# siyuanwu99/pred-occ-planner

Hardware: AMD Instinct MI355X
Metric: replans/sec (SOGM update + QP: full replan = SOGM update + A* + corridors + QP + deconfliction), 128-agent batch per GPU, 200x200x200x20 voxel grid; aggregate over all agents (higher is better)
Workload: dtype f32 occupancy / f64 planning; 1 GPU; 128 agents/GPU x 1 GPU, 200x200x200x20 SOGM, sim_fkpcp-style moving cylinders, batched ADMM QP (BASELINE configs[2] per GPU); agents_total=128, cloud_points=622040, cylinders=555, map_input_staleness_ticks=0, parallelism=agents sharded x1, 1 all-gather/tick, exchange=local, sogm_grids_per_agent=3, sogm_reset=sparse (logged 32-byte sectors), sogm_cell_order=2x2x2 tiles, map_update=at the start of the tick

## Files before the change

### pred-occ-planner_amd/csrc/sogm_qp.hip

```cpp
#include <hip/hip_runtime.h>

#include <cstdlib>

#include "../../include/sogm_detmath.h"
#include "sogm_planner.hpp"
#include "sogm_qp_layout.hpp"

#include <type_traits>

namespace sogm {
namespace {

#define QP_NMAX (15 * SOGM_MAX_PIECES)
#define QP_NT 512
#define QP_K1_DOUBLES (15 * QP_FAST_MAX_PIECES * (QP_BW + 1))

__device__ const double OSQP_INFTY  = 1e30;
__device__ const double MIN_SCALING = 1e-04, MAX_SCALING = 1e+04;
__device__ const double RHO_MIN = 1e-06, RHO_TOL = 1e-04, RHO_EQ_OVER_RHO_INEQ = 1e03;

__device__ inline double dabs(double x) { return x < 0 ? -x : x; }
__device__ inline double dmax(double a, double b) { return a > b ? a : b; }
__device__ inline double limit_scaling(double v) {
  v = v < MIN_SCALING ? 1.0 : v;
// ... 47 lines not shown
  v += dpp_ctrl_t<0x4E>(v);
  v += dpp_ctrl_t<0x141>(v);
  v += dpp_ctrl_t<0x140>(v);
  return (read_lane(v, 0) + read_lane(v, 16)) + (read_lane(v, 32) + read_lane(v, 48));
}
__device__ inline double block_max(double v, double *s_red) {
  v = wave_max(v);
  __syncthreads();
  if ((threadIdx.x & 63) == 0) s_red[threadIdx.x >> 6] = v;
  __syncthreads();
  return dmax(dmax(dmax(s_red[0], s_red[1]), dmax(s_red[2], s_red[3])),
              dmax(dmax(s_red[4], s_red[5]), dmax(s_red[6], s_red[7])));
}

static_assert(row_bytes('S', true) == (3 + 1) * sizeof(double) && row_bytes('G', true) == sizeof(double), "carve_rows: hot arrays");
static_assert(row_bytes('G', false) == (QP_ELL + 8) * sizeof(double) + 2 * QP_ELL * sizeof(int) &&
                  row_bytes('S', false) == 5 * sizeof(double) + sizeof(int),
              "carve_rows: cold arrays");
__device__ inline void carve_rows(Rows &R, char *hot, char *cold, int G, int S) {
  double *h = (double *)hot;
  R.sval = h;  h += (size_t)S * 3;
  R.sw = h;    h += S;
  R.gw = h;
  double *d = (double *)cold;
  R.gval = d;  d += (size_t)G * QP_ELL;
  R.gl = d;    d += G;
  R.gu = d;    d += G;
  R.grho = d;  d += G;
  R.gE = d;    d += G;
  R.gz = d;    d += G;
  R.gy = d;    d += G;
  R.gdy = d;   d += G;
  R.grinv = d; d += G;
  R.su = d;    d += S;
  R.sE = d;    d += S;
  R.sz = d;    d += S;
  R.sy = d;    d += S;
  R.sdy = d;   d += S;
  int *q = (int *)d;
  R.gcol = q;  q += (size_t)G * QP_ELL;
  R.sc0 = q;   q += S;
  R.cidx = q;
}

#define dpp_quad(v, ctrl) dpp_ctrl_t<ctrl>(v)

__device__ inline int launder(int v) {
  asm volatile("" : "+v"(v));
  return v;
}

__device__ inline double &KB(double *Kb, int i, int j) { return Kb[i * (QP_BW + 1) + (i - j)]; }

}

__device__ __forceinline__ void qp_solve_agent(const SogmPlannerParams &pp, const SogmQpSettings &qs,
                                               const QpWorkspace &ws, const QpConst &qc, const QpIO &io,
                                               int ablate_arg, int agent) {
#ifdef SOGM_QP_ABLATE_BUILD
  const int ablate = ablate_arg;
#else
  constexpr int ablate = 0;
  (void)ablate_arg;
#endif
  const int tid = threadIdx.x, lane = tid & 63, wave = tid >> 6;
  const long long dbg_t0 = wall_clock64(), dbg_clk0 = clock64();
  long long       dbg_refac = 0, dbg_check = 0, dbg_f1 = 0, dbg_f2 = 0, dbg_f3 = 0, dbg_k1 = 0, dbg_k2 = 0;
  int             dbg_nrefac = 0, dbg_ncheck = 0;
  const int M = io.npoly[agent];
  if (M <= 0 || M > SOGM_MAX_PIECES) {
    if (tid == 0) {
      io.out_status[agent] = -100;
      io.out_iters[agent]  = 0;
    }
    return;
  }
  const int MF = pp.max_faces;
  const int n  = 15 * M;

  extern __shared__ __attribute__((aligned(16))) char qp_smem[];
  const bool use_blocks = M <= QP_FAST_MAX_PIECES;
  __shared__ double s_ginv[QP_NMAX];
  __shared__ __attribute__((aligned(16))) double s_xt[QP_NMAX];
  __shared__ double s_x[QP_NMAX], s_D[QP_NMAX], s_Dt[QP_NMAX];
  __shared__ __attribute__((aligned(16))) double s_cn[QP_NMAX];
  __shared__ double s_red[8];
  __shared__ double s_T[2][225];
  __shared__ double s_red12[96];
  __shared__ double s_sc[16];
  __shared__ int    s_off[SOGM_MAX_PIECES + 1];
  __shared__ int    s_nf[SOGM_MAX_PIECES];
  __shared__ int    s_cnt[QP_NMAX + 1];
  __shared__ int    s_cptr[QP_NMAX + 1];
  __shared__ int    s_flag;

  if (tid == 0) {
    int acc = 0;
    for (int i = 0; i < M; ++i) {
      const int f = io.nfaces[agent * SOGM_MAX_PIECES + i];
      s_off[i]    = acc;
      s_nf[i]     = f;
      acc += 5 * f;
    }
    s_off[M] = acc;
  }
  __syncthreads();
// ... 234 lines not shown
      }
      R.gE[r] *= et;
    }
    for (int s = tid; s < S; s += QP_NT) {
      double      *v  = R.sval + (size_t)s * 3;
      const double mx = __builtin_fmax(__builtin_fmax(__builtin_fabs(v[0]), __builtin_fabs(v[1])), __builtin_fabs(v[2]));
      const double et = 1.0 / sogm_det::sqrt_rn(limit_scaling(mx));
      const int    c0 = R.sc0[s];
      v[0] *= et * s_Dt[c0];
      v[1] *= et * s_Dt[c0 + 1];
      v[2] *= et * s_Dt[c0 + 2];
      R.sE[s] *= et;
    }
    for (int jq = launder(tid); jq < 4 * n; jq += QP_NT) {
      const int     j = jq >> 2, q = jq & 3, b15 = (j / 15) * 15;
      double       *Pb = s_P + (j / 15) * 225 + j % 15;
      const double  dj = s_Dt[j];
      double        mx = 0;
      for (int i = q; i < 15; i += 4) {
        const double v = (Pb[i * 15] * ct_prev) * (s_Dt[b15 + i] * dj);
        Pb[i * 15]     = v;
        mx             = __builtin_fmax(mx, __builtin_fabs(v));
      }
      mx = __builtin_fmax(mx, dpp_quad(mx, 0xB1));
      mx = __builtin_fmax(mx, dpp_quad(mx, 0x4E));
      if (q == 0) {
        s_cn[j] = mx;
        s_D[j] *= dj;
      }
    }
    __syncthreads();
    if (tid == 0) {
      double mean = 0;
      for (int j = 0; j < n; ++j) mean += s_cn[j];
      double c_temp = mean / n;
      c_temp        = dmax(c_temp, limit_scaling(0.0));
      c_temp        = limit_scaling(c_temp);
      s_sc[0]       = 1.0 / c_temp;
    }
    __syncthreads();
    ct_prev = s_sc[0];
    c_scale *= ct_prev;
  }
  for (int i = tid; i < M * 225; i += QP_NT) s_P[i] *= ct_prev;
  for (int r = tid; r < G; r += QP_NT) {
    R.gl[r] *= R.gE[r];
    R.gu[r] *= R.gE[r];
  }
  for (int s = tid; s < S; s += QP_NT) R.su[s] *= R.sE[s];
  const double cinv = 1.0 / c_scale;
  __syncthreads();
  const long long dbg_s2 = wall_clock64() - dbg_t0;

  double rho_cur = qs.rho;
  double rinv_cur = 1.0 / rho_cur;
  double    kinv[30] = {};
  auto   set_rho = [&]() {
    const int tid = launder((int)threadIdx.x), lane = tid & 63, wave = tid >> 6;
    (void)lane;
    (void)wave;
    for (int r = tid; r < G; r += QP_NT) {
      const double lo = R.gl[r], hi = R.gu[r];
      double       v;
      if (lo < -OSQP_INFTY * MIN_SCALING && hi > OSQP_INFTY * MIN_SCALING)
        v = RHO_MIN;
      else if (hi - lo < RHO_TOL)
        v = RHO_EQ_OVER_RHO_INEQ * rho_cur;
      else
        v = rho_cur;
      R.grho[r]  = v;
      R.grinv[r] = 1.0 / v;
    }
    for (int s = tid; s < S; s += QP_NT) R.sw[s] = rho_cur * R.sz[s] - R.sy[s];
    __syncthreads();
  };
  auto build_K1 = [&]() {
    const int tid = launder((int)threadIdx.x);
    for (int e = tid; e < n * (QP_BW + 1); e += QP_NT) {
      const int i = e / (QP_BW + 1), dlt = e % (QP_BW + 1), j = i - dlt;
      double    s = 0.0;
      if (j >= 0) {
        for (int a = s_cptr[i]; a < s_cptr[i + 1]; ++a) {
          const int    en = R.cidx[a], r = en >> 3;
          const double vi = R.gval[(size_t)r * QP_ELL + (en & 7)];
          const double mr = R.gu[r] - R.gl[r] < RHO_TOL ? RHO_EQ_OVER_RHO_INEQ : 1.0;
          for (int k = 0; k < QP_ELL; ++k)
            if (R.gcol[(size_t)r * QP_ELL + k] == j) s += vi * mr * R.gval[(size_t)r * QP_ELL + k];
        }
        if (i / 3 == j / 3) {
          COL_DECODE(i)
          const int jd = j % 3;
          for (int f = 0; f < nface; ++f) {
            const double *v = R.sval + (size_t)(sbase + 5 * f) * 3;
            s += v[pd] * v[jd];
          }
        }
      }
      k1w[e] = s;
    }
    __threadfence_block();
    __syncthreads();
  };
  auto factor = [&]() __attribute__((always_inline)) -> bool {
    const int tid = launder((int)threadIdx.x), lane = tid & 63, wave = tid >> 6;
    (void)lane;
    (void)wave;
    if constexpr (FAST) {
      const long long dbg_fa = wall_clock64();
      for (int e = tid; e < 2 * M * 225; e += QP_NT) {
        const int which = e >= M * 225 ? 1 : 0, ee = e - which * M * 225;
        const int b = ee / 225, r = (ee % 225) / 15, c = ee % 15;
        int       i = b * 15 + r, j = (b - which) * 15 + c;
        double    s = 0.0;
        if (j >= 0) {
          if (i < j) {
            const int t_ = i;
            i            = j;
            j            = t_;
          }
          if (i / 15 == j / 15) s = s_P[(i / 15) * 225 + (i % 15) * 15 + (j % 15)];
          if (i == j) s += qs.sigma;
          if (i - j <= QP_BW) s = __builtin_fma(rho_cur, k1r[i * (QP_BW + 1) + (i - j)], s);
        }
        (which ? s_V : s_Dv)[ee] = s;
      }
      if (tid == 0) s_flag = 1;
      __syncthreads();
      const long long dbg_fb = wall_clock64();
      dbg_f1 += dbg_fb - dbg_fa;
      const int  er = (tid % 225) / 15, ec = tid % 15;
      const bool el = tid < 225;
      const int  hi_ = er > ec ? er : ec, lo_ = er > ec ? ec : er;
      for (int i = 0; i < M; ++i) {
        double a = 0.0;
        if (i > 0) {
          if (el) {
            const double *Or = s_V + i * 225 + er * 15, *Dc = s_Dv + (i - 1) * 225 + ec;
            double        t  = 0.0;
#pragma unroll
            for (int k = 0; k < 15; ++k) t = __builtin_fma(Or[k], Dc[k * 15], t);
            s_T[0][tid] = t;
          }
          __syncthreads();
          if (el) {
            const double *Tr = s_T[0] + hi_ * 15, *Oc = s_V + i * 225 + lo_ * 15;
            double        t  = s_Dv[i * 225 + hi_ * 15 + lo_];
#pragma unroll
            for (int k = 0; k < 15; ++k) t = __builtin_fma(-Tr[k], Oc[k], t);
            a = t;
          }
          __syncthreads();
          if (el) s_V[i * 225 + tid] = s_T[0][tid];
        } else if (el) {
// ... 279 lines not shown
    }
    if (!(ablate & 64))
    for (int j = tid; j < n; j += QP_NT) {
      double        s  = 0;
      const double *Pb = s_P + (j / 15) * 225 + (j % 15) * 15;
      const int     b0 = (j / 15) * 15;
      for (int k = 0; k < 15; ++k) s += Pb[k] * s_x[b0 + k];
      const double a  = col_sum_y(j);
      const double dj = 1.0 / s_D[j];
      m[3]            = dmax(m[3], dabs(dj * (s + a)));
      m[4]            = dmax(m[4], dabs(dj * s));
      m[5]            = dmax(m[5], dabs(dj * a));
      m[9]            = dmax(m[9], dabs(s + a));
      m[10]           = dmax(m[10], dabs(s));
      m[11]           = dmax(m[11], dabs(a));
    }
    if (!(ablate & 128))
#pragma unroll
    for (int k = 0; k < 12; ++k) m[k] = wave_max(m[k]);
    __syncthreads();
    if (lane == 0) {
      double *o = s_red12 + wave * 12;
#pragma unroll
      for (int k = 0; k < 12; ++k) o[k] = m[k];
    }
    __syncthreads();
    if (tid < 12) {
      double v = s_red12[tid];
      for (int w = 1; w < QP_NT / 64; ++w) v = dmax(v, s_red12[12 * w + tid]);
      s_sc[tid < 6 ? tid : tid + 2] = tid == 3 ? v * cinv : v;
    }
    if (tid == 12) s_sc[6] = s_sc[14] = 0.0;
    __syncthreads();
  };

  double *const h_sv = (double *)(qp_smem + head);
  double *const h_sw = h_sv + (size_t)S * 3;
  double *const h_gw = h_sw + S;
  double rs[24];
  int    ri[QP_ELL];
#define gv(k) rs[k]
#define gc(k) ri[k]
#define g_rho rs[6]
#define g_rinv rs[7]
#define g_lo rs[8]
#define g_hi rs[9]
#define g_z rs[10]
#define g_y rs[11]
#define sv(u, d) rs[6 * (u) + (d)]
#define s_hi(u) rs[6 * (u) + 3]
#define s_zr(u) rs[6 * (u) + 4]
#define s_yr(u) rs[6 * (u) + 5]
#define s_c(u) ri[u]
  double cv[2], xj = 0.0;
  int    cr[2];
#pragma unroll
  for (int k = 0; k < 24; ++k) rs[k] = 0.0;
#pragma unroll
  for (int k = 0; k < QP_ELL; ++k) ri[k] = 0;
  cv[0] = cv[1] = 0.0;
  cr[0] = cr[1] = 0;
  const bool grole = tid < 256;
  const bool grow = tid < G, ccol = tid < 4 * n;
  int        fj_sv = 0, fj_sw = 0, fj_n = 0;
  auto fast_load = [&]() __attribute__((always_inline)) {
    const int t  = launder(tid);
    const int tg = grow ? t : 0;
    if (grole) {
#pragma unroll
      for (int k = 0; k < QP_ELL; ++k) {
        const int    c = R.gcol[(size_t)tg * QP_ELL + k];
        const double v = R.gval[(size_t)tg * QP_ELL + k];
        gc(k)          = (c < 0 || !grow) ? 0 : c;
        gv(k)          = (c < 0 || !grow) ? 0.0 : v;
      }
      g_lo = R.gl[tg];
      g_hi = R.gu[tg];
      g_z  = R.gz[tg];
      g_y  = R.gy[tg];
#pragma unroll
      for (int k = 12; k < 24; ++k) rs[k] = 0.0;
    } else {
#pragma unroll
      for (int u = 0; u < 4; ++u) {
        const int  sr = (t - 256) + 256 * u;
        const bool ok = sr < S;
        const int  sc = ok ? sr : 0;
        const double a0 = R.sval[(size_t)sc * 3 + 0], a1 = R.sval[(size_t)sc * 3 + 1], a2 = R.sval[(size_t)sc * 3 + 2];
        const double hi = R.su[sc], z = R.sz[sc], y = R.sy[sc];
        const int    c0 = R.sc0[sc];
        sv(u, 0) = ok ? a0 : 0.0;
        sv(u, 1) = ok ? a1 : 0.0;
        sv(u, 2) = ok ? a2 : 0.0;
        s_hi(u)  = ok ? hi : 0.0;
        s_zr(u)  = ok ? z : 0.0;
        s_yr(u)  = ok ? y : 0.0;
        s_c(u)   = ok ? c0 : 0;
      }
      ri[4] = ri[5] = 0;
    }
    {
      const int j = ccol ? t >> 2 : 0, q = t & 3;
#pragma unroll
      for (int e = 0; e < 2; ++e) {
        const int    qq = s_cptr[j] + q + 4 * e;
        const bool   ok = ccol && qq < s_cptr[j + 1];
        const int    en = R.cidx[ok ? qq : s_cptr[j]];
        const double v  = R.gval[(size_t)(en >> 3) * QP_ELL + (en & 7)];
        cr[e]           = ok ? en >> 3 : 0;
        cv[e]           = ok ? v : 0.0;
      }
      COL_DECODE(j)
      fj_sv = (sbase + 5 * q) * 3 + pd;
      fj_sw = sbase + 5 * q;
      fj_n  = ccol ? (nface - q + 3) >> 2 : 0;
      xj    = s_x[j];
    }
  };
  auto fast_rho = [&]() __attribute__((always_inline)) {
    const int t  = launder(tid);
    const int tg = grow ? t : 0;
    if (grole) {
      g_rho  = R.grho[tg];
      g_rinv = R.grinv[tg];
      if (grow) h_gw[t] = g_rho * g_z - g_y;
    }
  };
  double *const c_sy = (double *)qp_smem + (size_t)M * 225;
  double *const c_gy = c_sy + S;
  double *const c_red = c_gy + G;
  auto fast_stage_y = [&]() __attribute__((always_inline)) {
    const int t = launder(tid);
    if (grole) {
      if (grow) c_gy[t] = g_y;
    } else {
#pragma unroll
      for (int u = 0; u < 4; ++u) {
        const int sr = (t - 256) + 256 * u;
        if (sr < S) c_sy[sr] = s_yr(u);
      }
    }
    if (ccol && (t & 3) == 0) s_x[t >> 2] = xj;
    __syncthreads();
  };
  auto fast_spill = [&]() __attribute__((always_inline)) {
    const int t = launder(tid);
    if (grole) {
      if (grow) {
        R.gz[t] = g_z;
        R.gy[t] = g_y;
      }
    } else {
#pragma unroll
      for (int u = 0; u < 4; ++u) {
        const int sr = (t - 256) + 256 * u;
        if (sr < S) {
          R.sz[sr] = s_zr(u);
          R.sy[sr] = s_yr(u);
        }
      }
    }
    if (ccol && (t & 3) == 0) s_x[t >> 2] = xj;
    __syncthreads();
  };

  auto cert_stage1 = [&]() {
    const int tid = launder((int)threadIdx.x), lane = tid & 63, wave = tid >> 6;
    double    ndy = 0, lhs = 0;
    for (int r = tid; r < G; r += QP_NT) {
      const double d = R.gdy[r];
      ndy            = dmax(ndy, dabs(R.gE[r] * d));
      lhs += R.gu[r] * (d > 0 ? d : 0) + R.gl[r] * (d < 0 ? d : 0);
    }
    for (int s = tid; s < S; s += QP_NT) {
      const double d = R.sdy[s] > 0.0 ? R.sdy[s] : 0.0;
      R.sdy[s]       = d;
      ndy            = dmax(ndy, dabs(R.sE[s] * d));
      lhs += R.su[s] * d;
    }
    ndy = block_max(ndy, s_red);
    lhs = wave_sum(lhs);
    __syncthreads();
    if (lane == 0) s_red[wave] = lhs;
    __syncthreads();
    if (tid == 0) {
      s_sc[7]  = ndy;
      s_sc[15] = ((s_red[0] + s_red[1]) + (s_red[2] + s_red[3])) + ((s_red[4] + s_red[5]) + (s_red[6] + s_red[7]));
    }
    __syncthreads();
  };
  auto primal_infeasible = [&](double eps_inf) -> bool {
    const int tid = launder((int)threadIdx.x);
    if constexpr (!FAST) cert_stage1();
    const double ndy = s_sc[7], lhs = s_sc[15];
    if (!(ndy > eps_inf)) return false;
    if (!(lhs < -eps_inf * ndy)) return false;
    double na = 0;
    if constexpr (FAST) {
      if (ccol) {
        const int     j = tid >> 2;
        double        a = __builtin_fma(cv[1], R.gdy[cr[1]], cv[0] * R.gdy[cr[0]]);
        const double *fvp = h_sv + fj_sv, *fyp = R.sdy + fj_sw;
        const double *fv0 = fvp, *fy0 = fyp;
#pragma unroll 1
        for (int i0 = 0; i0 < fj_n; i0 += 4, fvp += 240, fyp += 80) {
          double av[4], bv[4];
#pragma unroll
          for (int u = 0; u < 4; ++u) {
            const bool ok = i0 + u < fj_n;
            av[u]         = *(ok ? fvp + 60 * u : fv0);
            bv[u]         = *(ok ? fyp + 20 * u : fy0);
            bv[u]         = ok ? bv[u] : 0.0;
          }
#pragma unroll
          for (int u = 0; u < 4; ++u) a = __builtin_fma(av[u], bv[u], a);
        }
        a += dpp_quad(a, 0xB1);
        a += dpp_quad(a, 0x4E);
        na = dabs((1.0 / s_D[j]) * a);
      }
    } else {
      for (int j = tid; j < n; j += QP_NT) {
        double a = 0;
        for (int q = s_cptr[j]; q < s_cptr[j + 1]; ++q) {
          const int en = R.cidx[q], r = en >> 3;
          a += R.gval[(size_t)r * QP_ELL + (en & 7)] * R.gdy[r];
        }
        COL_DECODE(j)
        for (int f = 0; f < nface; ++f) {
          const int sr = sbase + 5 * f;
          a += R.sval[(size_t)sr * 3 + pd] * R.sdy[sr];
        }
        na = dmax(na, dabs((1.0 / s_D[j]) * a));
      }
    }
    na = block_max(na, s_red);
    __syncthreads();
    return na < eps_inf * ndy;
  };

  auto fast_residuals = [&]() __attribute__((always_inline)) {
    const int  t = launder(tid), lane = t & 63, wave = t >> 6;
    const bool f32 = qs.residual_fp32 != 0;
    auto fab = [](double x) __attribute__((always_inline)) { return __builtin_fabs(x); };
    auto fmx = [](double a, double b) __attribute__((always_inline)) { return __builtin_fmax(a, b); };
    double    v[10];
#pragma unroll
    for (int k = 0; k < 10; ++k) v[k] = 0.0;
    if (grole) {
      double xg[QP_ELL];
#pragma unroll
      for (int k = 0; k < QP_ELL; ++k) xg[k] = s_x[gc(k)];
      const int    tg = grow ? t : 0;
      const double e = R.gE[tg], d = R.gdy[tg];
      double       ax = 0.0;
#pragma unroll
      for (int k = 0; k < QP_ELL; ++k) ax += gv(k) * xg[k];
      if (grow) {
        const double r_ = fab(ax - g_z), n_ = fmx(fab(ax), fab(g_z));
        const double ei = 1.0 / e;
        v[0] = f32 ? (double)((float)r_ / (float)e) : ei * r_;
        v[1] = f32 ? (double)((float)n_ / (float)e) : ei * n_;
        v[2] = r_;
        v[3] = n_;
        v[8] = fab(e * d);
        v[9] = g_hi * (d > 0 ? d : 0) + g_lo * (d < 0 ? d : 0);
      }
    } else {
      double se[4], sd[4];
#pragma unroll
      for (int u = 0; u < 4; ++u) {
        const int sr = (t - 256) + 256 * u, sc = sr < S ? sr : 0;
        se[u] = R.sE[sc];
        sd[u] = R.sdy[sc];
      }
#pragma unroll
      for (int u = 0; u < 4; ++u) {
        if (256 * u >= S) continue;
        const int    sr = (t - 256) + 256 * u;
        const bool   ok = sr < S;
        const double x0 = s_x[s_c(u)], x1 = s_x[s_c(u) + 1], x2 = s_x[s_c(u) + 2];
        const double e = se[u], dr_ = sd[u];
        double       ax = 0.0;
        ax += sv(u, 0) * x0;
        ax += sv(u, 1) * x1;
        ax += sv(u, 2) * x2;
        if (ok) {
          const double d  = dr_ > 0.0 ? dr_ : 0.0;
          R.sdy[sr]       = d;
          const double r_ = fab(ax - s_zr(u)), n_ = fmx(fab(ax), fab(s_zr(u)));
          const double ei = 1.0 / e;
          v[0] = fmx(v[0], f32 ? (double)((float)r_ / (float)e) : ei * r_);
          v[1] = fmx(v[1], f32 ? (double)((float)n_ / (float)e) : ei * n_);
          v[2] = fmx(v[2], r_);
          v[3] = fmx(v[3], n_);
          v[8] = fmx(v[8], fab(e * d));
          v[9] += s_hi(u) * d;
        }
      }
    }
    if (ccol) {
      const int     j = t >> 2, q = t & 3, b0 = (j / 15) * 15;
      const double *Pb = s_P + (j / 15) * 225 + (j % 15) * 15;
      double        pk[4], xk[4], yg[2];
#pragma unroll
      for (int u = 0; u < 4; ++u) {
        const int k = q + 4 * u, kk = k < 15 ? k : 0;
        pk[u]       = Pb[kk];
        xk[u]       = s_x[b0 + kk];
      }
#pragma unroll
      for (int e = 0; e < 2; ++e) yg[e] = c_gy[cr[e]];
      double        s_ = 0.0, a_ = 0.0;
      {
        const double *fvp = h_sv + fj_sv, *fyp = c_sy + fj_sw;
        const double *fv0 = fvp, *zero = s_xt + 127;
#pragma unroll 1
        for (int i0 = 0; i0 < fj_n; i0 += 4, fvp += 240, fyp += 80) {
          double a[4], b[4];
#pragma unroll
          for (int u = 0; u < 4; ++u) {
            const bool ok = i0 + u < fj_n;
            a[u]          = *(ok ? fvp + 60 * u : fv0);
            b[u]          = *(ok ? fyp + 20 * u : zero);
          }
          __builtin_amdgcn_sched_barrier(0);
#pragma unroll
          for (int u = 0; u < 4; ++u) a_ = __builtin_fma(a[u], b[u], a_);
        }
      }
#pragma unroll
      for (int u = 0; u < 4; ++u) s_ = __builtin_fma(q + 4 * u < 15 ? pk[u] : 0.0, xk[u], s_);
#pragma unroll
      for (int e = 0; e < 2; ++e) a_ = __builtin_fma(cv[e], yg[e], a_);
      s_ += dpp_quad(s_, 0xB1);
      a_ += dpp_quad(a_, 0xB1);
      s_ += dpp_quad(s_, 0x4E);
      a_ += dpp_quad(a_, 0x4E);
      if (q == 0) {
        const double dj = s_D[j], di = 1.0 / dj;
        const double r_ = fab(s_ + a_), n_ = fmx(fab(s_), fab(a_));
        v[4] = f32 ? (double)((float)r_ / (float)dj) : di * r_;
        v[5] = f32 ? (double)((float)n_ / (float)dj) : di * n_;
        v[6] = r_;
        v[7] = n_;
      }
    }
    if (f32) {
#pragma unroll
      for (int k = 0; k < 9; ++k) {
        float fv = (float)v[k];
        if ((double)fv < v[k]) fv = __int_as_float(__float_as_int(fv) + 1);
        v[k] = (double)fv;
      }
    }
#pragma unroll
    for (int k = 0; k < 9; ++k) {
      double x = v[k];
      x        = __builtin_fmax(x, dpp_ctrl_t<0xB1>(x));
      x        = __builtin_fmax(x, dpp_ctrl_t<0x4E>(x));
      x        = __builtin_fmax(x, dpp_ctrl_t<0x141>(x));
      v[k]     = __builtin_fmax(x, dpp_ctrl_t<0x140>(x));
    }
    {
      double x = v[9];
      x += dpp_ctrl_t<0xB1>(x);
      x += dpp_ctrl_t<0x4E>(x);
      x += dpp_ctrl_t<0x141>(x);
      v[9] = x + dpp_ctrl_t<0x140>(x);
    }
    if ((lane & 15) == 0) {
      double *o = c_red + (wave * 4 + (lane >> 4)) * 10;
#pragma unroll
      for (int k = 0; k < 10; ++k) o[k] = v[k];
    }
    __syncthreads();
    if (t < 40) {
      const int     k = t >> 2, pq = t & 3;
      const double *o = c_red + (size_t)(8 * pq) * 10 + k;
      double        r_;
      if (k == 9) {
        r_ = ((o[0] + o[10]) + (o[20] + o[30])) + ((o[40] + o[50]) + (o[60] + o[70]));
        r_ += dpp_quad(r_, 0xB1);
        r_ += dpp_quad(r_, 0x4E);
      } else {
        r_ = __builtin_fmax(__builtin_fmax(__builtin_fmax(o[0], o[10]), __builtin_fmax(o[20], o[30])),
                            __builtin_fmax(__builtin_fmax(o[40], o[50]), __builtin_fmax(o[60], o[70])));
        r_ = __builtin_fmax(r_, dpp_quad(r_, 0xB1));
        r_ = __builtin_fmax(r_, dpp_quad(r_, 0x4E));
      }
      const int slot = k == 0 ? 0 : k == 1 ? 1 : k == 2 ? 8 : k == 3 ? 9 : k == 4 ? 3 : k == 5 ? 4 : k == 6 ? 11 : k == 7 ? 12 : k == 8 ? 7 : 15;
      if (pq == 0) s_sc[slot] = k == 4 ? r_ * cinv : r_;
    }
    if (t >= 64 && t < 70)
      s_sc[t == 64 ? 2 : t == 65 ? 5 : t == 66 ? 6 : t == 67 ? 10 : t == 68 ? 13 : 14] = 0.0;
    __syncthreads();
  };

  set_rho();
  if constexpr (FAST) build_K1();
  const long long dbg_s3 = wall_clock64() - dbg_t0;
  bool chol_ok = factor();
  const long long dbg_setup = wall_clock64() - dbg_t0;
  int  status = -2, iter = 0;
  if (!chol_ok) status = -7;
  if constexpr (FAST) {
    fast_load();
    fast_rho();
    __syncthreads();
  }

  int cj_q0 = 0, cj_q1 = 0, cj_sbase = 0, cj_nface = 0, cj_pd = 0;
  if (tid < n) {
    COL_DECODE(tid)
    cj_q0    = s_cptr[tid];
    cj_q1    = s_cptr[tid + 1];
    cj_sbase = sbase;
    cj_nface = nface;
    cj_pd    = pd;
  }
  double alpha = qs.alpha, oma = 1.0 - qs.alpha, sigma_v = qs.sigma;
  asm volatile("" : "+v"(alpha), "+v"(oma), "+v"(sigma_v));
  const double *xtv   = FAST ? s_cn : s_xt;
  for (int j = n + tid; j < 128; j += QP_NT) s_xt[j] = 0.0;
  __syncthreads();
  auto iteration = [&](auto store_tag, auto ns_tag) __attribute__((always_inline)) {
      constexpr bool STORE = decltype(store_tag)::value;
      constexpr int  NS    = decltype(ns_tag)::value;
      (void)NS;
      if constexpr (FAST) {
        if (!(ablate & 1) && ccol) {
          double w[2];
#pragma unroll
          for (int e = 0; e < 2; ++e) w[e] = h_gw[cr[e]];
          double        p   = 0.0;
          const double *fvp = h_sv + fj_sv, *fwp = h_sw + fj_sw;
          const double *fv0 = fvp, *zero = s_xt + 127;
#pragma unroll 1
          for (int i0 = 0; i0 < fj_n; i0 += 4, fvp += 240, fwp += 80) {
            double a[4], b[4];
#pragma unroll
            for (int u = 0; u < 4; ++u) {
              const bool ok = i0 + u < fj_n;
              a[u]          = *(ok ? fvp + 60 * u : fv0);
              b[u]          = *(ok ? fwp + 20 * u : zero);
            }
            __builtin_amdgcn_sched_barrier(0);
#pragma unroll
            for (int u = 0; u < 4; ++u) p = __builtin_fma(a[u], b[u], p);
          }
#pragma unroll
          for (int e = 0; e < 2; ++e) p = __builtin_fma(cv[e], w[e], p);
          p += dpp_quad(p, 0xB1);
          p += dpp_quad(p, 0x4E);
          if ((tid & 3) == 0) s_xt[launder(tid) >> 2] = __builtin_fma(sigma_v, xj, p);
        }
      } else
      if (!(ablate & 1))
      if (tid < n) {
        const int j = tid;
        double    s = qs.sigma * s_x[j];
        for (int q = cj_q0; q < cj_q1; ++q) {
          const int en = R.cidx[q], r = en >> 3;
          s += R.gval[(size_t)r * QP_ELL + (en & 7)] * (R.grho[r] * R.gz[r] - R.gy[r]);
        }
        const double *sv = R.sval + (size_t)cj_sbase * 3 + cj_pd;
        const double *sw = R.sw + cj_sbase;
        for (int f = 0; f < cj_nface; ++f) s += sv[(size_t)15 * f] * sw[5 * f];
        s_xt[j] = s;
      }
      __syncthreads();
      if (!(ablate & 2)) solveK();
      if constexpr (FAST) {
        if (!(ablate & 12)) {
          const int    t   = launder(tid);
          const double xtj = xtv[ccol ? t >> 2 : 0];
          if (grole) {
            double xg[QP_ELL];
#pragma unroll
            for (int k = 0; k < QP_ELL; ++k) xg[k] = xtv[gc(k)];
            __builtin_amdgcn_sched_barrier(0);
            double s = gv(0) * xg[0];
#pragma unroll
            for (int k = 1; k < QP_ELL; ++k) s = __builtin_fma(gv(k), xg[k], s);
            const double zr = __builtin_fma(alpha, s, oma * g_z);
            double       v  = __builtin_fma(g_rinv, g_y, zr);
            v               = __builtin_fmin(__builtin_fmax(v, g_lo), g_hi);
            g_z             = v;
            const double d  = g_rho * (zr - v);
            g_y             = g_y + d;
            if (grow) {
              h_gw[t] = __builtin_fma(g_rho, v, -g_y);
              if constexpr (STORE) R.gdy[t] = d;
            }
          } else {
            double xs[NS][3];
#pragma unroll
            for (int u = 0; u < NS; ++u) {
              xs[u][0] = xtv[s_c(u)];
              xs[u][1] = xtv[s_c(u) + 1];
              xs[u][2] = xtv[s_c(u) + 2];
            }
            __builtin_amdgcn_sched_barrier(0);
#pragma unroll
            for (int u = 0; u < NS; ++u) {
              double ax = sv(u, 0) * xs[u][0];
              ax              = __builtin_fma(sv(u, 1), xs[u][1], ax);
              ax              = __builtin_fma(sv(u, 2), xs[u][2], ax);
              const double zr = __builtin_fma(alpha, ax, oma * s_zr(u));
              double       v  = __builtin_fma(rinv_cur, s_yr(u), zr);
              v               = __builtin_fmin(v, s_hi(u));
              s_zr(u)         = v;
              const double d  = rho_cur * (zr - v);
              const double yn = s_yr(u) + d;
              s_yr(u)         = yn;
              const int sr    = (t - 256) + 256 * u;
              if (u + 1 < NS || sr < S) {
                h_sw[sr] = __builtin_fma(rho_cur, v, -yn);
                if constexpr (STORE) R.sdy[sr] = d;
              }
            }
          }
          xj = __builtin_fma(alpha, xtj, oma * xj);
        }
        __syncthreads();
      } else {
      if (!(ablate & 4))
      for (int r = tid; r < G; r += QP_NT) {
        double s = 0;
        for (int k = 0; k < QP_ELL; ++k) {
          const int c = R.gcol[(size_t)r * QP_ELL + k];
          if (c >= 0) s += R.gval[(size_t)r * QP_ELL + k] * xtv[c];
        }
        const double rho = R.grho[r], yr = R.gy[r];
        const double zr  = alpha * s + (1.0 - alpha) * R.gz[r];
        double       v   = zr + R.grinv[r] * yr;
        const double lo = R.gl[r], hi = R.gu[r];
        v               = v < lo ? lo : (v > hi ? hi : v);
        R.gz[r]         = v;
        const double d  = rho * (zr - v);
        R.gdy[r]        = d;
        R.gy[r]         = yr + d;
      }
      if (!(ablate & 8))
      for (int s = tid; s < S; s += QP_NT) {
        const int     c0 = R.sc0[s];
        const double *vv = R.sval + (size_t)s * 3;
        double        ax = 0;
        ax += vv[0] * xtv[c0];
        ax += vv[1] * xtv[c0 + 1];
        ax += vv[2] * xtv[c0 + 2];
        const double yr = R.sy[s];
        const double zr = alpha * ax + (1.0 - alpha) * R.sz[s];
        double       v  = zr + rinv_cur * yr;
        const double hi = R.su[s];
        v               = v > hi ? hi : v;
        R.sz[s]         = v;
        const double d  = rho_cur * (zr - v);
        R.sdy[s]        = d;
        const double yn = yr + d;
        R.sy[s]         = yn;
        R.sw[s]         = rho_cur * v - yn;
      }
      for (int j = tid; j < n; j += QP_NT) s_x[j] = alpha * xtv[j] + (1.0 - alpha) * s_x[j];
      __syncthreads();
      }
  };
  int adapt_left = qs.adaptive_rho_interval, check_left = qs.check_termination;
  bool finished = !chol_ok;
  if (chol_ok) {
    const int max_iter = qs.max_iter, adapt_iv = qs.adaptive_rho_interval, check_iv = qs.check_termination;
// ... 89 lines not shown
      } else {
        residuals();
      }
      const double eps_prim = qs.eps_abs * 10 + qs.eps_rel * 10 * dmax(s_sc[1], s_sc[2]);
      const double eps_dual =
          qs.eps_abs * 10 + qs.eps_rel * 10 * cinv * dmax(dmax(s_sc[4], s_sc[5]), s_sc[6]);
      const bool p_ok = s_sc[0] < eps_prim;
      if (p_ok && s_sc[3] < eps_dual)
        status = 2;
      else if (!p_ok && primal_infeasible(1e-4 * 10))
        status = 3;
      else
        status = -2;
    }
  }
  __syncthreads();
  double *out = io.out_cpts + (size_t)agent * SOGM_MAX_PIECES * 15;
  for (int j = tid; j < SOGM_MAX_PIECES * 15; j += QP_NT) out[j] = j < n ? s_D[j] * s_x[j] : 0.0;
  if (tid == 0) {
    io.out_status[agent] = status;
    io.out_iters[agent]  = iter;
    if (ws.dbg) {
      long long *o = ws.dbg + (size_t)agent * SOGM_QP_STAT_N;
      o[SOGM_QP_STAT_FACTOR_ASM]    = dbg_f1;
      o[SOGM_QP_STAT_FACTOR_FWD]    = dbg_f2;
      o[SOGM_QP_STAT_FACTOR_BWD]    = dbg_f3;
      o[SOGM_QP_STAT_SHADER_CLOCKS] = clock64() - dbg_clk0;
      o[SOGM_QP_STAT_CHECK_STAGE]   = dbg_k1;
      o[SOGM_QP_STAT_CHECK_RESID]   = dbg_k2;
      o[SOGM_QP_STAT_TOTAL]         = wall_clock64() - dbg_t0;
      o[SOGM_QP_STAT_SETUP_SPLIT]   = dbg_s1 | (dbg_s2 << 20) | (dbg_s3 << 40);
      o[SOGM_QP_STAT_SETUP]         = dbg_setup;
      o[SOGM_QP_STAT_REFAC]         = dbg_refac;
      o[SOGM_QP_STAT_N_REFAC]       = dbg_nrefac;
      o[SOGM_QP_STAT_CHECK]         = dbg_check;
      o[SOGM_QP_STAT_N_CHECK]       = dbg_ncheck;
      o[SOGM_QP_STAT_ITERS]         = iter;
      o[SOGM_QP_STAT_PATH]          = (FAST ? 1 : 0) | (rows_in_lds ? 2 : 0);
    }
  }
#undef gv
#undef gc
#undef g_rho
#undef g_rinv
#undef g_lo
#undef g_hi
#undef g_z
#undef g_y
#undef sv
#undef s_hi
#undef s_zr
#undef s_yr
#undef s_c
  };
  using std::false_type;
  using std::true_type;
  if (rows_in_lds) {
    Rows R;
    carve_rows(R, qp_smem + head, qp_smem + head + rows_hot_bytes(G, S), G, S);
    if (fast)
      body(R, true_type{});
    else
      body(R, false_type{});
  } else {
    char *scr = ws.scratch + (size_t)agent * ws.scratch_stride;
    Rows  R;
    carve_rows(R, fast ? qp_smem + head : scr, scr + rows_hot_bytes(G, S), G, S);
    if (fast)
      body(R, true_type{});
    else
      body(R, false_type{});
  }
}

__global__ __launch_bounds__(QP_NT) void k_qp(SogmPlannerParams pp, SogmQpSettings qs, QpWorkspace ws,
                                            QpConst qc, const double *__restrict__ start_pva,
                                            const double *__restrict__ goal_pv,
                                            const double *__restrict__ polys,
                                            const int32_t *__restrict__ nfaces,
                                            const int32_t *__restrict__ npoly,
                                            double *__restrict__ out_cpts,
                                            int32_t *__restrict__ out_status,
                                            int32_t *__restrict__ out_iters, int ablate_arg, int agent0) {
  const QpIO io{.start_pva = start_pva, .goal_pv = goal_pv, .polys = polys, .nfaces = nfaces, .npoly = npoly,
                .out_cpts = out_cpts, .out_status = out_status, .out_iters = out_iters};
  qp_solve_agent(pp, qs, ws, qc, io, ablate_arg, blockIdx.x + agent0);
}

__global__ __launch_bounds__(QP_NT) void k_qp_flow(SogmPlannerParams pp, SogmQpSettings qs, QpWorkspace ws,
                                                 QpConst qc, FlowCtl fc, QpIO io, int ablate_arg, int n_agents) {
  __shared__ int s_agent;
  if (threadIdx.x == 0) atomicAdd(&fc.hdr[FLOW_Q_RESIDENT], 1);
  for (;;) {
    if (threadIdx.x == 0) {
      int       a = -1;
      const int k = atomicAdd(&fc.hdr[FLOW_Q_TICKET], 1);
      if (k < n_agents) a = wait_at_least<WaitQpItem, false>(&fc.hdr[FLOW_ERR], fc.q_ready + k, 0);
      s_agent = a;
    }
    __syncthreads();
    const int agent = __builtin_amdgcn_readfirstlane(s_agent);
    if (agent < 0) break;
    __threadfence();
    if (threadIdx.x == 0) fc.ts[agent * 8 + 4] = wall_clock64();
    qp_solve_agent(pp, qs, ws, qc, io, ablate_arg, agent);
    __syncthreads();
// ... 69 lines not shown
```

### pred-occ-planner_amd/csrc/sogm_qp_layout.hpp

```cpp
#pragma once
#include <cstddef>
#include "../../include/sogm_abi.h"
#ifdef __HIPCC__
#include <hip/hip_runtime.h>
#define QP_HD __host__ __device__ __forceinline__
#define QP_HDI __host__ __device__ inline
#else
#define QP_HD inline
#define QP_HDI inline
#endif

namespace sogm {

constexpr int QP_BW  = 17;
constexpr int QP_ELL = 6;

struct QpShape {
  int M, n;
  int R1, R3, R4;
  int G, S;
  QP_HD QpShape(int pieces, int faces)
      : M(pieces), n(15 * pieces), R1(3 * (pieces + 1)), R3(9 * (pieces + 1)), R4(R3 + 12 * pieces), G(R4 + 9 * pieces),
        S(5 * faces) {}
};

#define QP_ROW_ARRAYS(X)                                                                                      \
  X(sval, S, 3, double, true)                                                            \
  X(sw, S, 1, double, true)          \
  X(gw, G, 1, double, true)                                                 \
  X(gval, G, QP_ELL, double, false)                                                           \
  X(gl, G, 1, double, false)                                                                                  \
  X(gu, G, 1, double, false)                                                                                  \
  X(grho, G, 1, double, false)                                                                                \
  X(gE, G, 1, double, false)                                                                                  \
  X(gz, G, 1, double, false)                                                                                  \
  X(gy, G, 1, double, false)                                                                                  \
  X(gdy, G, 1, double, false)                                                                                 \
  X(grinv, G, 1, double, false)                                               \
  X(su, S, 1, double, false)                                                                                  \
  X(sE, S, 1, double, false)                                                                                  \
  X(sz, S, 1, double, false)                                                                                  \
  X(sy, S, 1, double, false)                                                                                  \
  X(sdy, S, 1, double, false)                                                                                 \
  X(gcol, G, QP_ELL, int, false)                                              \
  X(sc0, S, 1, int, false)                                       \
  X(cidx, G, QP_ELL, int, false)

struct Rows {
#define X(name, rows, per, T, hot) T *name;
  QP_ROW_ARRAYS(X)
#undef X
};

constexpr size_t row_bytes(char of, bool want_hot) {
  constexpr char G = 'G', S = 'S';
  size_t         b = 0;
#define X(name, rows, per, T, hot) \
  if (rows == of && hot == want_hot) b += per * sizeof(T);
  QP_ROW_ARRAYS(X)
#undef X
  return b;
}
static_assert(row_bytes('S', true) % sizeof(double) == 0 && row_bytes('G', true) % sizeof(double) == 0, "the hot arrays hold doubles");
QP_HDI size_t rows_hot_bytes(int G, int S) {
  return ((size_t)S * (row_bytes('S', true) / sizeof(double)) + G * (row_bytes('G', true) / sizeof(double))) * sizeof(double);
}
QP_HDI size_t rows_cold_bytes(int G, int S) {
  return (size_t)G * row_bytes('G', false) + (size_t)S * row_bytes('S', false) + 64;
}
QP_HDI size_t rows_bytes(int G, int S) { return rows_hot_bytes(G, S) + rows_cold_bytes(G, S); }

constexpr int QP_FAST_MAX_PIECES = 8;
constexpr int QP_FAST_MAX_G = 256;
constexpr int QP_FAST_MAX_S = 1024;
constexpr int QP_CHECK_RED = 32 * 10;

struct QpLayout {
// ... 44 lines not shown
```

Before: 12890 replans/s.

## Store sval and sw in column-major runs for contiguous column dot products

After building K1 in the fast QP path, the safety-face constraint values (sval) are permuted into a column-major layout grouped by piece, coordinate and face residue. The ADMM w-vector (sw) is written in the same order. Per-column dot products then read contiguous runs and can use paired 2-wide vector loads through a new run_dot helper, instead of strided loads (stride 60/20). This adds a one-time permutation pass with an extra barrier, extra index-decode arithmetic, and packed write offsets kept in registers.

```diff
diff --git a/pred-occ-planner_amd/csrc/sogm_qp.hip b/pred-occ-planner_amd/csrc/sogm_qp.hip
--- a/pred-occ-planner_amd/csrc/sogm_qp.hip
+++ b/pred-occ-planner_amd/csrc/sogm_qp.hip
@@ -123,6 +123,52 @@
 
 __device__ inline double &KB(double *Kb, int i, int j) { return Kb[i * (QP_BW + 1) + (i - j)]; }
 
+constexpr int QP_RUN_PAIRS = 5;
+typedef double qp_d2 __attribute__((ext_vector_type(2)));
+typedef qp_d2 qp_d2u __attribute__((aligned(8)));
+template <int K>
+__device__ __forceinline__ void run_load(qp_d2 (&a)[QP_RUN_PAIRS], qp_d2 (&b)[QP_RUN_PAIRS], const double *fv,
+                                         const double *fw, int left) {
+  a[K] = *(const qp_d2u *)(fv + 2 * K);
+  b[K] = *(const qp_d2u *)(fw + 2 * K);
+  if constexpr (K + 1 < QP_RUN_PAIRS)
+    if (left > K + 1) run_load<K + 1>(a, b, fv, fw, left);
+}
+template <int K>
+__device__ __forceinline__ double run_fma(const qp_d2 (&a)[QP_RUN_PAIRS], const qp_d2 (&b)[QP_RUN_PAIRS], int left,
+                                          double p) {
+  p = __builtin_fma(a[K].x, b[K].x, p);
+  p = __builtin_fma(a[K].y, b[K].y, p);
+  if constexpr (K + 1 < QP_RUN_PAIRS)
+    if (left > K + 1) {
+      asm volatile("");
+      p = run_fma<K + 1>(a, b, left, p);
+    }
+  return p;
+}
+__device__ __forceinline__ double run_batch(const double *fv, const double *fw, int left, double p) {
+  qp_d2 a[QP_RUN_PAIRS], b[QP_RUN_PAIRS];
+#pragma unroll
+  for (int k = 1; k < QP_RUN_PAIRS; ++k) asm volatile("" : "=v"(a[k]), "=v"(b[k]));
+  run_load<0>(a, b, fv, fw, left);
+  __builtin_amdgcn_sched_barrier(0);
+  return run_fma<0>(a, b, left, p);
+}
+__device__ __forceinline__ double run_dot(const double *fv, const double *fw, int nrun, const double *zero, double p) {
+  const bool   odd = nrun & 1;
+  const int    np  = nrun >> 1;
+  const double ta = *(odd ? fv + (nrun - 1) : zero), tb = *(odd ? fw + (nrun - 1) : zero);
+  if (np > 0) {
+    p = run_batch(fv, fw, np, p);
+    if (np > QP_RUN_PAIRS) {
+#pragma unroll 1
+      for (int i0 = QP_RUN_PAIRS; i0 < np; i0 += QP_RUN_PAIRS)
+        p = run_batch(fv + 2 * i0, fw + 2 * i0, np - i0, p);
+    }
+  }
+  return __builtin_fma(ta, tb, p);
+}
+
 }
 
 __device__ __forceinline__ void qp_solve_agent(const SogmPlannerParams &pp, const SogmQpSettings &qs,
@@ -463,6 +509,18 @@
   __syncthreads();
   const long long dbg_s2 = wall_clock64() - dbg_t0;
 
+  auto row_decode = [&](int s, int &off, int &nf, int &f, int &cp) __attribute__((always_inline)) {
+    const int c0 = R.sc0[s], i = c0 / 15;
+    cp  = (c0 - 15 * i) / 3;
+    off = s_off[i];
+    nf  = s_nf[i];
+    f   = (s - off - cp) / 5;
+  };
+  auto sw_pos = [&](int s) __attribute__((always_inline)) -> int {
+    int off, nf, f, cp;
+    row_decode(s, off, nf, f, cp);
+    return qp_colmajor(off, nf, f, cp, 0, 1);
+  };
   double rho_cur = qs.rho;
   double rinv_cur = 1.0 / rho_cur;
   double    kinv[30] = {};
@@ -482,7 +540,7 @@
       R.grho[r]  = v;
       R.grinv[r] = 1.0 / v;
     }
-    for (int s = tid; s < S; s += QP_NT) R.sw[s] = rho_cur * R.sz[s] - R.sy[s];
+    for (int s = tid; s < S; s += QP_NT) R.sw[FAST ? sw_pos(s) : s] = rho_cur * R.sz[s] - R.sy[s];
     __syncthreads();
   };
   auto build_K1 = [&]() {
@@ -510,6 +568,28 @@
       k1w[e] = s;
     }
     __threadfence_block();
+    __syncthreads();
+  };
+  static_assert(3 * QP_FAST_MAX_S <= 6 * QP_NT, "colmajor_sval: six elements per lane");
+  auto colmajor_sval = [&]() {
+    const int tid = launder((int)threadIdx.x);
+    double    v[6];
+#pragma unroll
+    for (int k = 0; k < 6; ++k) {
+      const int e = tid + QP_NT * k;
+      v[k]        = R.sval[e < 3 * S ? e : 0];
+    }
+    __syncthreads();
+#pragma unroll
+    for (int k = 0; k < 6; ++k) {
+      const int e = tid + QP_NT * k;
+      if (e < 3 * S) {
+        const int s = e / 3;
+        int       off, nf, f, cp;
+        row_decode(s, off, nf, f, cp);
+        R.sval[qp_colmajor(off, nf, f, cp, e - 3 * s, 3)] = v[k];
+      }
+    }
     __syncthreads();
   };
   auto factor = [&]() __attribute__((always_inline)) -> bool {
@@ -895,6 +975,7 @@
 #define s_zr(u) rs[6 * (u) + 4]
 #define s_yr(u) rs[6 * (u) + 5]
 #define s_c(u) ri[u]
+#define s_wd(u) ((ri[4 + ((u) >> 1)] >> (16 * ((u) & 1))) & 0xFFFF)
   double cv[2], xj = 0.0;
   int    cr[2];
 #pragma unroll
@@ -924,12 +1005,16 @@
 #pragma unroll
       for (int k = 12; k < 24; ++k) rs[k] = 0.0;
     } else {
+      int wd[4];
 #pragma unroll
       for (int u = 0; u < 4; ++u) {
         const int  sr = (t - 256) + 256 * u;
         const bool ok = sr < S;
         const int  sc = ok ? sr : 0;
-        const double a0 = R.sval[(size_t)sc * 3 + 0], a1 = R.sval[(size_t)sc * 3 + 1], a2 = R.sval[(size_t)sc * 3 + 2];
+        int        off, nf, f, cp;
+        row_decode(sc, off, nf, f, cp);
+        const double *vp = R.sval + qp_colmajor(off, nf, f, cp, 0, 3);
+        const double  a0 = vp[0], a1 = vp[nf], a2 = vp[2 * nf];
         const double hi = R.su[sc], z = R.sz[sc], y = R.sy[sc];
         const int    c0 = R.sc0[sc];
         sv(u, 0) = ok ? a0 : 0.0;
@@ -939,8 +1024,10 @@
         s_zr(u)  = ok ? z : 0.0;
         s_yr(u)  = ok ? y : 0.0;
         s_c(u)   = ok ? c0 : 0;
-      }
-      ri[4] = ri[5] = 0;
+        wd[u]    = qp_colmajor(off, nf, f, cp, 0, 1) * (int)sizeof(double);
+      }
+      ri[4] = wd[0] | wd[1] << 16;
+      ri[5] = wd[2] | wd[3] << 16;
     }
     {
       const int j = ccol ? t >> 2 : 0, q = t & 3;
@@ -954,8 +1041,9 @@
         cv[e]           = ok ? v : 0.0;
       }
       COL_DECODE(j)
-      fj_sv = (sbase + 5 * q) * 3 + pd;
-      fj_sw = sbase + 5 * q;
+      (void)sbase;
+      fj_sv = qp_colmajor(s_off[pi], nface, q, pk, pd, 3);
+      fj_sw = qp_colmajor(s_off[pi], nface, q, pk, 0, 1);
       fj_n  = ccol ? (nface - q + 3) >> 2 : 0;
       xj    = s_x[j];
     }
@@ -980,7 +1068,7 @@
 #pragma unroll
       for (int u = 0; u < 4; ++u) {
         const int sr = (t - 256) + 256 * u;
-        if (sr < S) c_sy[sr] = s_yr(u);
+        if (sr < S) *(double *)((char *)c_sy + s_wd(u)) = s_yr(u);
       }
     }
     if (ccol && (t & 3) == 0) s_x[t >> 2] = xj;
@@ -1043,15 +1131,17 @@
       if (ccol) {
         const int     j = tid >> 2;
         double        a = __builtin_fma(cv[1], R.gdy[cr[1]], cv[0] * R.gdy[cr[0]]);
-        const double *fvp = h_sv + fj_sv, *fyp = R.sdy + fj_sw;
+        COL_DECODE(j)
+        (void)nface;
+        const double *fvp = h_sv + fj_sv, *fyp = R.sdy + sbase + 5 * (tid & 3);
         const double *fv0 = fvp, *fy0 = fyp;
 #pragma unroll 1
-        for (int i0 = 0; i0 < fj_n; i0 += 4, fvp += 240, fyp += 80) {
+        for (int i0 = 0; i0 < fj_n; i0 += 4, fvp += 4, fyp += 80) {
           double av[4], bv[4];
 #pragma unroll
           for (int u = 0; u < 4; ++u) {
             const bool ok = i0 + u < fj_n;
-            av[u]         = *(ok ? fvp + 60 * u : fv0);
+            av[u]         = *(ok ? fvp + u : fv0);
             bv[u]         = *(ok ? fyp + 20 * u : fy0);
             bv[u]         = ok ? bv[u] : 0.0;
           }
@@ -1155,23 +1245,7 @@
 #pragma unroll
       for (int e = 0; e < 2; ++e) yg[e] = c_gy[cr[e]];
       double        s_ = 0.0, a_ = 0.0;
-      {
-        const double *fvp = h_sv + fj_sv, *fyp = c_sy + fj_sw;
-        const double *fv0 = fvp, *zero = s_xt + 127;
-#pragma unroll 1
-        for (int i0 = 0; i0 < fj_n; i0 += 4, fvp += 240, fyp += 80) {
-          double a[4], b[4];
-#pragma unroll
-          for (int u = 0; u < 4; ++u) {
-            const bool ok = i0 + u < fj_n;
-            a[u]          = *(ok ? fvp + 60 * u : fv0);
-            b[u]          = *(ok ? fyp + 20 * u : zero);
-          }
-          __builtin_amdgcn_sched_barrier(0);
-#pragma unroll
-          for (int u = 0; u < 4; ++u) a_ = __builtin_fma(a[u], b[u], a_);
-        }
-      }
+      a_ = run_dot(h_sv + fj_sv, c_sy + fj_sw, fj_n, s_xt + 127, a_);
 #pragma unroll
       for (int u = 0; u < 4; ++u) s_ = __builtin_fma(q + 4 * u < 15 ? pk[u] : 0.0, xk[u], s_);
 #pragma unroll
@@ -1241,7 +1315,10 @@
   };
 
   set_rho();
-  if constexpr (FAST) build_K1();
+  if constexpr (FAST) {
+    build_K1();
+    colmajor_sval();
+  }
   const long long dbg_s3 = wall_clock64() - dbg_t0;
   bool chol_ok = factor();
   const long long dbg_setup = wall_clock64() - dbg_t0;
@@ -1276,22 +1353,7 @@
           double w[2];
 #pragma unroll
           for (int e = 0; e < 2; ++e) w[e] = h_gw[cr[e]];
-          double        p   = 0.0;
-          const double *fvp = h_sv + fj_sv, *fwp = h_sw + fj_sw;
-          const double *fv0 = fvp, *zero = s_xt + 127;
-#pragma unroll 1
-          for (int i0 = 0; i0 < fj_n; i0 += 4, fvp += 240, fwp += 80) {
-            double a[4], b[4];
-#pragma unroll
-            for (int u = 0; u < 4; ++u) {
-              const bool ok = i0 + u < fj_n;
-              a[u]          = *(ok ? fvp + 60 * u : fv0);
-              b[u]          = *(ok ? fwp + 20 * u : zero);
-            }
-            __builtin_amdgcn_sched_barrier(0);
-#pragma unroll
-            for (int u = 0; u < 4; ++u) p = __builtin_fma(a[u], b[u], p);
-          }
+          double p = run_dot(h_sv + fj_sv, h_sw + fj_sw, fj_n, s_xt + 127, 0.0);
 #pragma unroll
           for (int e = 0; e < 2; ++e) p = __builtin_fma(cv[e], w[e], p);
           p += dpp_quad(p, 0xB1);
@@ -1359,7 +1421,7 @@
               s_yr(u)         = yn;
               const int sr    = (t - 256) + 256 * u;
               if (u + 1 < NS || sr < S) {
-                h_sw[sr] = __builtin_fma(rho_cur, v, -yn);
+                *(double *)((char *)h_sw + s_wd(u)) = __builtin_fma(rho_cur, v, -yn);
                 if constexpr (STORE) R.sdy[sr] = d;
               }
             }
@@ -1555,6 +1617,7 @@
 #undef s_zr
 #undef s_yr
 #undef s_c
+#undef s_wd
   };
   using std::false_type;
   using std::true_type;
diff --git a/pred-occ-planner_amd/csrc/sogm_qp_layout.hpp b/pred-occ-planner_amd/csrc/sogm_qp_layout.hpp
--- a/pred-occ-planner_amd/csrc/sogm_qp_layout.hpp
+++ b/pred-occ-planner_amd/csrc/sogm_qp_layout.hpp
@@ -23,6 +23,11 @@
       : M(pieces), n(15 * pieces), R1(3 * (pieces + 1)), R3(9 * (pieces + 1)), R4(R3 + 12 * pieces), G(R4 + 9 * pieces),
         S(5 * faces) {}
 };
+
+QP_HD int qp_colmajor_run(int nf, int q) { return (nf >> 2) * q + ((nf & 3) < q ? (nf & 3) : q); }
+QP_HD int qp_colmajor(int off, int nf, int f, int cp, int d, int per) {
+  return per * off + (per * cp + d) * nf + qp_colmajor_run(nf, f & 3) + (f >> 2);
+}
 
 #define QP_ROW_ARRAYS(X)                                                                                      \
   X(sval, S, 3, double, true)                                                            \
```

Result: no change. 12900 replans/s, median of 2 (+0.0%).
